# AndrewCullacino/handwritten-chinese-ocr-samples

Hardware: AMD Instinct MI355X
Metric: text-lines/sec (1x128x2000 synth) greedy decode (higher is better)
Workload: dtype f16 (f32 accumulate); 1 GPU; BASELINE configs[1]: 64 x 1x128x2000 uint8 lines, random-init hctr checkpoint (C=7358), forward + greedy CTC decode, labels to host; global_lines=64, lines_per_gpu=64, width=2000, classes=7358, checkpoint=random, parallelism=batch-shard x1

## Files before the change

handwritten-chinese-ocr-samples_amd/csrc/kernels.hip:

```cpp
#include "kernels.h"

#include <algorithm>
#include <climits>
#include <cstdlib>

namespace hctr {

typedef _Float16 f16x8 __attribute__((ext_vector_type(8)));
typedef float f32x4 __attribute__((ext_vector_type(4)));
typedef float f32x2 __attribute__((ext_vector_type(2)));
typedef _Float16 f16x2 __attribute__((ext_vector_type(2)));
typedef uint32_t u32x4 __attribute__((ext_vector_type(4)));
typedef void __attribute__((address_space(3))) * lptr_t;

__device__ __forceinline__ void glds16_asm(const char* gsrc, char* lds_dst) {
    const uint32_t lds = (uint32_t)(uintptr_t)((lptr_t)lds_dst);
    uint32_t keep;
    asm volatile("s_mov_b32 %0, m0\n\ts_mov_b32 m0, %2\n\ts_nop 0\n\tglobal_load_lds_dwordx4 %1, off\n\ts_mov_b32 m0, %0"
                 : "=&s"(keep)
                 : "v"(gsrc), "s"(lds)
                 : "memory");
}

template <int CTRL>
// ... 562 lines not shown
#pragma unroll
                    for (int n = 0; n < 4; ++n) dst[n] = *(const f16x8*)(xt + n * 2048 + (ks ? foff1 : foff0));
                };
                __builtin_amdgcn_sched_barrier(0);
                read_b(0, bq[0]);
                read_a(0, ar[0]);
                __builtin_amdgcn_sched_barrier(0);
                read_a(1, ar[1]);
                __builtin_amdgcn_sched_barrier(0);
                if (k + 1 < nk) stage(k + 1, (k + 1) & 1);
                __builtin_amdgcn_sched_barrier(0);
#pragma unroll
                for (int g = 0; g < 8; ++g) {
                    if (g + 2 < 8) read_a(g + 2, ar[(g + 2) % 3]);
                    __builtin_amdgcn_sched_barrier(0);
                    if (g == 1) { read_b(1, bq[1]); __builtin_amdgcn_sched_barrier(0); }
                    __builtin_amdgcn_s_setprio(1);
#pragma unroll
                    for (int jj = 0; jj < 2; ++jj)
#pragma unroll
                        for (int n = 0; n < 4; ++n)
                            acc[2 * (g & 3) + jj][n] = __builtin_amdgcn_mfma_f32_16x16x32_f16(ar[g % 3][jj], bq[g >> 2][n],
                                                                                             acc[2 * (g & 3) + jj][n], 0, 0, 0);
                    __builtin_amdgcn_s_setprio(0);
                    __builtin_amdgcn_sched_barrier(0);
                }
                continue;
            }
            if (k + 1 < nk) stage(k + 1, (k + 1) & 1);
#pragma unroll
            for (int ks = 0; ks < 2; ++ks) {
                const int fo = ks ? foff1 : foff0;
                f16x8 af[JT], bf[4];
#pragma unroll
                for (int n = 0; n < 4; ++n) bf[n] = *(const f16x8*)(xt + n * 2048 + fo);
#pragma unroll
                for (int j = 0; j < JT; ++j) af[j] = *(const f16x8*)(wt + j * 2048 + fo);
                __builtin_amdgcn_s_setprio(1);
#pragma unroll
                for (int j = 0; j < JT; ++j)
#pragma unroll
                    for (int n = 0; n < 4; ++n)
                        acc[j][n] = __builtin_amdgcn_mfma_f32_16x16x32_f16(af[j], bf[n], acc[j][n], 0, 0, 0);
                __builtin_amdgcn_s_setprio(0);
            }
        }
    } else {
        constexpr int NG = 2 * JT;
        constexpr int NP = NIW + NIX;
        for (int k = 0; k < nk; ++k) {
            asm volatile("s_waitcnt vmcnt(0)" ::: "memory");
            __syncthreads();
            const int kn = k + 1 < nk ? k + 1 : k;
            int64_t wo_n, xo_n;
            step_offsets(kn, wo_n, xo_n);
            const char* wsrc_n = wbase + wo_n;
            const char* xsrc_n = xbase + xo_n;
            const int buf_n = (k + 1) & 1;
            const char* wt = smem + (k & 1) * TILE_BYTES + (wn * WC) * 128;
            const char* xt = smem + (k & 1) * TILE_BYTES + BN * 128 + (wm * 64) * 128;
            f16x8 bfr[2][4], afr[2];
#pragma unroll
            for (int n = 0; n < 4; ++n) bfr[0][n] = *(const f16x8*)(xt + n * 2048 + foff0);
            afr[0] = *(const f16x8*)(wt + foff0);
#pragma unroll
            for (int g = 0; g < NG; ++g) {
                const int ks = g / JT, j = g % JT;
                if (g + 1 < NG) {
                    const int ks1 = (g + 1) / JT, j1 = (g + 1) % JT;
                    afr[(g + 1) & 1] = *(const f16x8*)(wt + j1 * 2048 + (ks1 ? foff1 : foff0));
                }
                if (g == JT / 2) {
#pragma unroll
                    for (int n = 0; n < 4; ++n) bfr[1][n] = *(const f16x8*)(xt + n * 2048 + foff1);
                }
                if ((g * NP) / NG != ((g + 1) * NP) / NG)
                    stage_piece(wsrc_n, xsrc_n, buf_n, (g * NP) / NG);
#pragma unroll
                for (int n = 0; n < 4; ++n)
                    acc[j][n] = __builtin_amdgcn_mfma_f32_16x16x32_f16(afr[g & 1], bfr[ks][n], acc[j][n], 0, 0, 0);
                __builtin_amdgcn_sched_barrier(0);
            }
        }
    }

    conv_epilogue<WN, WM, JT, LINEAR, SPLIT>(a, acc, smem, tid, lane, wn, wm, n0, mt, img, th, tw,
                                             th * (4 * WM) + wm * 4, tw * kTileW);
}

static int env_dbg() {
    if (getenv("HCTR_DBG_LAYER")) return 0;
    const char* e = getenv("HCTR_DBG");
    return e ? atoi(e) : 0;
}

static hipError_t raise_lds_limit(const void* fn, int bytes, bool (&done)[64]) {
    int dev = 0;
    hipError_t e = hipGetDevice(&dev);
    if (e != hipSuccess) return e;
    if (dev < 0 || dev >= 64) return hipErrorInvalidDevice;
    if (done[dev]) return hipSuccess;
    e = hipFuncSetAttribute(fn, hipFuncAttributeMaxDynamicSharedMemorySize, bytes);
    if (e == hipSuccess) done[dev] = true;
    return e;
}

constexpr int kHaloCols = 20;
constexpr int kHaloRows = 18;
constexpr int kHaloBytes = kHaloRows * kHaloCols * 128;
constexpr int kHaloPieces = kHaloRows * kHaloCols / 8;
constexpr int kHaloLds = 2 * 32768 + 2 * kHaloBytes;

template <bool SPLIT>
__global__ __launch_bounds__(512) void conv3x3_halo_kernel(const ConvArgs a) {
    constexpr int WN = 2, WM = 4, JT = 8, BN = 256;
    extern __shared__ __attribute__((aligned(16))) char smem[];
    const int tid = threadIdx.x;
    const int lane = tid & 63;
    const int wv = __builtin_amdgcn_readfirstlane(tid >> 6);
    const int wn = wv / WM, wm = wv % WM;

    const int total = a.mtiles * a.ntiles;
    int lin;
    {
        const int id = blockIdx.x, xcd = id & 7, s = id >> 3;
        const int q = total >> 3, r = total & 7;
        lin = (xcd < r ? xcd * (q + 1) : r * (q + 1) + (xcd - r) * q) + s;
    }
    const int nt = lin % a.ntiles;
    const int mt = lin / a.ntiles;
    const int n0 = nt * BN;
    const int tw = mt % a.tilesW;
    const int t2 = mt / a.tilesW;
    const int th = t2 % a.tilesH;
    const int img = t2 / a.tilesH;
    const int cin = a.Cin;
    const int nkc = cin / kBK;

    const char* xbase = (const char*)(a.x + img * a.in_sb + (int64_t)(th * 16) * a.in_sh + (int64_t)(tw * 16) * cin);
    const char* wbase = (const char*)(a.w + (int64_t)n0 * cin);
    const bool loader = wv < 4;
    uint32_t woff[8], hoff[12];
#pragma unroll
    for (int i = 0; i < 8; ++i) {
        const int g = ((wv & 3) * 8 + i) * 64 + lane;
        const int row = g >> 3, cp = (g & 7) ^ (row & 7);
        woff[i] = (uint32_t)row * (uint32_t)cin * 2u + cp * 16;
    }
#pragma unroll
    for (int r = 0; r < 12; ++r) {
        const int piece = ((r >> 1) * 4 + (wv & 3)) * 2 + (r & 1);
        const int g = piece * 64 + lane;
        const int row = g >> 3, cp = (g & 7) ^ (row & 7);
        int hy = row / kHaloCols, hx = row - hy * kHaloCols;
        if (hx > 17) hx = 17;
        if (hy > 17) hy = 17;
        hoff[r] = ((uint32_t)hy * (uint32_t)a.in_sh + (uint32_t)hx * (uint32_t)cin) * 2u + cp * 16;
    }
    const int q = lane >> 4, c = lane & 15;
    const int aoff0 = c * 128 + (((0 + q) ^ (lane & 7)) << 4);
    const int aoff1 = c * 128 + (((4 + q) ^ (lane & 7)) << 4);

    auto stage_weights = [&](int kc, int tap, int buf) {
        const char* src = wbase + ((int64_t)tap * a.CoutPad * cin + (int64_t)kc * kBK) * 2;
        char* dst = smem + buf * 32768 + ((wv & 3) * 8) * 1024;
#pragma unroll
        for (int i = 0; i < 8; ++i)
            glds16_asm(src + woff[i], dst + i * 1024);
    };
    auto stage_halo_piece = [&](int kc, int buf, int piece, uint32_t off) {
        if (piece < kHaloPieces) {
            const char* src = xbase + (int64_t)kc * (kBK * 2);
            char* dst = smem + 65536 + buf * kHaloBytes + piece * 1024;
            glds16_asm(src + off, dst);
        }
    };

    f32x4 acc[JT][4];
#pragma unroll
    for (int j = 0; j < JT; ++j)
#pragma unroll
        for (int n = 0; n < 4; ++n) acc[j][n] = (f32x4){0.f, 0.f, 0.f, 0.f};

    if (loader) {
#pragma unroll
        for (int r = 0; r < 12; ++r) stage_halo_piece(0, 0, ((r >> 1) * 4 + wv) * 2 + (r & 1), hoff[r]);
        stage_weights(0, 0, 0);
    }

    for (int kc = 0; kc < nkc; ++kc) {
        const bool next_chunk = kc + 1 < nkc;
        const int hbuf = 65536 + (kc & 1) * kHaloBytes + (wm * 4) * (kHaloCols * 128);
#pragma unroll 1
        for (int tap = 0; tap < 9; ++tap) {
            const int k = kc * 9 + tap;
            if (tap >= 1 && tap <= 5 && next_chunk) asm volatile("s_waitcnt vmcnt(2)" ::: "memory");
            else asm volatile("s_waitcnt vmcnt(0)" ::: "memory");
            __builtin_amdgcn_s_barrier();
            asm volatile("" ::: "memory");
            const int tdy = tap / 3, dx = tap - tdy * 3 - 1;
            const int u = c + 1 + dx;
            const int v0 = u * 128 + (((q ^ (u & 7) ^ ((tdy & 1) << 2)) & 7) << 4);
            const char* hb = smem + hbuf + tdy * (kHaloCols * 128);
            const char* be = hb + v0;
            const char* bo = hb + (v0 ^ 64);
            const char* wt = smem + (k & 1) * 32768 + (wn * 128) * 128;
            f16x8 ar[3][2], bq[2][4];
            auto read_a = [&](int g, f16x8 (&dst)[2]) {
                const int ks = g >> 2, jp = g & 3;
                const char* base = wt + (ks ? aoff1 : aoff0);
                dst[0] = *(const f16x8*)(base + (2 * jp) * 2048);
                dst[1] = *(const f16x8*)(base + (2 * jp + 1) * 2048);
            };
            auto read_b = [&](int ks, f16x8 (&dst)[4]) {
#pragma unroll
                for (int n = 0; n < 4; ++n)
                    dst[n] = *(const f16x8*)((((n & 1) ^ ks) ? bo : be) + n * (kHaloCols * 128));
            };
            __builtin_amdgcn_sched_barrier(0);
            read_b(0, bq[0]);
            read_a(0, ar[0]);
            __builtin_amdgcn_sched_barrier(0);
            read_a(1, ar[1]);
            __builtin_amdgcn_sched_barrier(0);
            if (loader) {
                int kc1 = kc, tap1 = tap + 1;
                if (tap1 == 9) { tap1 = 0; kc1 = next_chunk ? kc + 1 : kc; }
                if (a.dbg == 1) { kc1 = 0; tap1 = 0; }
                if (a.dbg != 2) stage_weights(kc1, tap1, (k + 1) & 1);
                if (next_chunk && tap < 6 && a.dbg != 2) {
                    uint32_t h0 = hoff[0], h1 = hoff[1];
                    h0 = tap == 1 ? hoff[2] : h0;  h1 = tap == 1 ? hoff[3] : h1;
                    h0 = tap == 2 ? hoff[4] : h0;  h1 = tap == 2 ? hoff[5] : h1;
                    h0 = tap == 3 ? hoff[6] : h0;  h1 = tap == 3 ? hoff[7] : h1;
                    h0 = tap == 4 ? hoff[8] : h0;  h1 = tap == 4 ? hoff[9] : h1;
                    h0 = tap == 5 ? hoff[10] : h0; h1 = tap == 5 ? hoff[11] : h1;
                    const int p0 = (tap * 4 + wv) * 2;
                    const int kcs = a.dbg == 1 ? 0 : kc + 1;
                    stage_halo_piece(kcs, (kc + 1) & 1, p0, h0);
                    stage_halo_piece(kcs, (kc + 1) & 1, p0 + 1, h1);
                }
            }
            __builtin_amdgcn_sched_barrier(0);
#pragma unroll
            for (int g = 0; g < 8; ++g) {
                const int ks = g >> 2, jp = g & 3;
                if (g + 2 < 8) read_a(g + 2, ar[(g + 2) % 3]);
                __builtin_amdgcn_sched_barrier(0);
                if (g == 1) { read_b(1, bq[1]); __builtin_amdgcn_sched_barrier(0); }
                __builtin_amdgcn_s_setprio(1);
#pragma unroll
                for (int jj = 0; jj < 2; ++jj)
#pragma unroll
                    for (int n = 0; n < 4; ++n)
                        acc[2 * jp + jj][n] = __builtin_amdgcn_mfma_f32_16x16x32_f16(ar[g % 3][jj], bq[ks][n],
                                                                                    acc[2 * jp + jj][n], 0, 0, 0);
                __builtin_amdgcn_s_setprio(0);
                __builtin_amdgcn_sched_barrier(0);
            }
        }
    }
    asm volatile("s_waitcnt vmcnt(0)" ::: "memory");
    conv_epilogue<WN, WM, JT, false, SPLIT>(a, acc, smem, tid, lane, wn, wm, n0, mt, img, th, tw, th * 16 + wm * 4,
                                            tw * 16);
}

namespace halo4_lds {
constexpr int kWeightBuf = 16384;
constexpr int kWeights = 0;
constexpr int kHalo = kWeights + 2 * kWeightBuf;
constexpr int kScratch = kHalo + kHaloBytes;
constexpr int kScratchBytes = 4 * 128 * 4;
constexpr int kHaloTable = kScratch;
constexpr int kHaloTableBytes = 4 * 12 * 8 * 4;
constexpr int kNextTile = kScratch + kScratchBytes;
constexpr int kTotal = kNextTile + 16;
static_assert(kHaloTableBytes <= kScratchBytes, "the halo-offset table fits inside the epilogue scratch it aliases");
static_assert(kNextTile >= kScratch + kScratchBytes, "the next-tile words lie behind the epilogue scratch");
static_assert(kTotal <= 80 * 1024, "two workgroups per CU on 160 KB of LDS");
}

template <int GEOM, bool SPLIT, bool PERSIST, bool STAMP = false, bool DSFUSE = false, bool RESPRE = false>
__global__ __launch_bounds__(256, 2) void conv3x3_halo4_kernel(const ConvArgs a) {
    static_assert(!DSFUSE || !PERSIST, "downsample fusion: non-persistent instances only");
    static_assert(!RESPRE || (!DSFUSE && !PERSIST && !SPLIT), "residual-in-prologue: plain f16 instances only");
    constexpr int WN = 1, WM = 4, JT = 8, BN = 128;
    constexpr int TR = GEOM ? 8 : 16, TC = GEOM ? 32 : 16;
    constexpr int S = TC + 4;
    static_assert((TR + 2) * S * 128 == kHaloBytes, "halo footprint");
    extern __shared__ __attribute__((aligned(16))) char smem[];
    const int tid = threadIdx.x;
    auto stamp = [&](int i) {
        if (STAMP && tid == 0) a.stamps[(size_t)blockIdx.x * 16 + i] = __builtin_amdgcn_s_memrealtime();
    };
    stamp(0);
    const int lane = tid & 63;
    const int wv = __builtin_amdgcn_readfirstlane(tid >> 6);
    const int wm = wv;
    const int cin = a.Cin;
    const int nkc = (a.dbg & 64) ? 0 : cin / kBK;
    const int nk = 9 * nkc;
    constexpr bool kPrefetch = !PERSIST && !STAMP && !RESPRE;
    static_assert(!(kPrefetch && PERSIST), "the halo-offset table aliases the epilogue scratch: one tile per workgroup");
    constexpr int kRing = 3;
    constexpr int kBhalfAt = 1;
    constexpr int kBpreAt = 4;
    constexpr int kEarlyAt = 1;

    {
        const int k0 = a.mtiles, k1 = a.ntiles, k2 = a.tilesW, k3 = a.tilesH, k4 = a.Cin, k5 = a.in_sh, k6 = a.nt_shift,
                  k7 = a.th_shift, k8 = a.CoutPad;
        const uint64_t k9 = a.tw_magic;
        const int64_t k10 = a.in_sb;
        const half_t *k11 = a.x, *k12 = a.w;
        const float* k13 = a.bias;
        asm volatile("" ::"s"(k0), "s"(k1), "s"(k2), "s"(k3), "s"(k4), "s"(k5), "s"(k6), "s"(k7), "s"(k8), "s"(k9), "s"(k10),
                     "s"(k11), "s"(k12), "s"(k13));
    }
    const int total = a.mtiles * a.ntiles;
    const int xcd = blockIdx.x & 7, local = blockIdx.x >> 3;
    const int tq = total >> 3, tr = total & 7;
    const int xbase_lin = xcd < tr ? xcd * (tq + 1) : tr * (tq + 1) + (xcd - tr) * tq;
    const int xcnt = tq + (xcd < tr ? 1 : 0);
    const int nloc = PERSIST ? (int)(gridDim.x >> 3) : 1;
    struct Tile { int n0, mt, img, th, tw; const char* xb; const char* wb; };
    auto tile_at = [&](int idx) {
        Tile t;
        const int lin = xbase_lin + idx;
        int nt, t2, th, img;
        if (a.nt_shift >= 0) { nt = lin & (a.ntiles - 1); t.mt = lin >> a.nt_shift; }
        else { nt = lin % a.ntiles; t.mt = lin / a.ntiles; }
        t.n0 = nt * BN;
        t2 = (int)(((uint64_t)(uint32_t)t.mt * a.tw_magic) >> 40);
        const int tw = t.mt - t2 * a.tilesW;
        if (a.th_shift >= 0) { th = t2 & (a.tilesH - 1); img = t2 >> a.th_shift; }
        else { th = t2 % a.tilesH; img = t2 / a.tilesH; }
        t.img = img; t.th = th; t.tw = tw;
        t.xb = (const char*)(a.x + img * a.in_sb + (int64_t)(th * TR) * a.in_sh + (int64_t)(tw * TC) * cin);
        t.wb = (const char*)(a.w + (int64_t)t.n0 * cin);
        return t;
    };
    int tidx = local;
    if (PERSIST && tidx >= xcnt) return;
    const bool dynamic = PERSIST && a.tile_counter != nullptr;
    int tnext = local + nloc;
    volatile int* lds_next = (volatile int*)(smem + halo4_lds::kNextTile);

    const int wrow = GEOM ? (wm >> 1) * 4 : wm * 4;
    const int wcol = GEOM ? (wm & 1) * 16 : 0;
    uint32_t woff[4], hoff[12];
    const int q = lane >> 4, c = lane & 15;
    const int aoff0 = c * 128 + (((0 + q) ^ (lane & 7)) << 4);
    const int aoff1 = c * 128 + (((4 + q) ^ (lane & 7)) << 4);

    auto weight_buf = [&](int k) { return smem + halo4_lds::kWeights + (k & 1) * halo4_lds::kWeightBuf; };
    auto stage_w = [&](const char* wb, int rowcin, const uint32_t (&wo)[4], int kc, int tap, int buf) {
        const char* src = wb + ((int64_t)tap * a.CoutPad * rowcin + (int64_t)kc * kBK) * 2;
        char* dst = weight_buf(buf) + (wv * 4) * 1024;
        const int64_t ps = (int64_t)rowcin * 16;
        glds16x4_asm_s(src, src + ps, src + 2 * ps, src + 3 * ps, wo[0], dst, dst + 1024, dst + 2048, dst + 3072);
    };
    auto stage_weights = [&](const char* wb, int kc, int tap, int buf) { stage_w(wb, cin, woff, kc, tap, buf); };
    auto stage_halo = [&](const char* xb, int kc) {
        const char* src = xb + (int64_t)kc * (kBK * 2);
#pragma unroll
        for (int r = 0; r < 12; ++r)
            if (wv + 4 * r < kHaloPieces) glds16_asm_s(src, hoff[r], smem + halo4_lds::kHalo + (wv + 4 * r) * 1024);
    };
    auto lane_offsets = [&](int rowcin, int in_sh, uint32_t (&wo)[4], bool with_halo) {
        int ln = lane;
        asm volatile("" : "+v"(ln));
#pragma unroll
        for (int i = 0; i < 4; ++i) {
            const int g = (wv * 4 + i) * 64 + ln;
            const int row = g >> 3, cp = (g & 7) ^ (row & 7);
            wo[i] = (uint32_t)row * (uint32_t)rowcin * 2u + cp * 16;
        }
        if (!with_halo) return;
#pragma unroll
        for (int r = 0; r < 12; ++r) {
            const int g = (wv + 4 * r) * 64 + ln;
            const int row = g >> 3, cp = (g & 7) ^ (row & 7);
            int hy = row / S, hx = row - hy * S;
            if (hx > TC + 1) hx = TC + 1;
            if (hy > TR + 1) hy = TR + 1;
            hoff[r] = ((uint32_t)hy * (uint32_t)in_sh + (uint32_t)hx * (uint32_t)rowcin) * 2u + cp * 16;
        }
    };
    auto write_halo_table = [&]() {
        uint32_t* htab = (uint32_t*)(smem + halo4_lds::kHaloTable);
        if ((lane & 7) == 0) {
            const uint32_t cp0 = (uint32_t)((lane >> 3) & 7) << 4;
#pragma unroll
            for (int r = 0; r < 12; ++r) htab[(wv * 12 + r) * 8 + (lane >> 3)] = hoff[r] - cp0;
        }
    };
    const int hbuf = halo4_lds::kHalo + wrow * (S * 128);
    int bx[3][2];
#pragma unroll
    for (int d = 0; d < 3; ++d) {
        const int u = wcol + c + d;
        const int v0 = u * 128 + (((q ^ (u & 7)) & 7) << 4);
        bx[d][0] = hbuf + v0;
        bx[d][1] = hbuf + (v0 ^ 64);
    }
    auto b_ptrs = [&](int tap, const char*& be, const char*& bo) {
        const int tdy = tap / 3, d = tap - tdy * 3;
        be = smem + bx[d][tdy & 1] + tdy * (S * 128);
        bo = smem + bx[d][(tdy & 1) ^ 1] + tdy * (S * 128);
    };

    Tile cur = tile_at(tidx);
    int kbase = 0;
    bool first = true;

    int tile_no = 0;
    for (;;) {
        const bool has_next = PERSIST && (tnext < xcnt);
        const char* nxb = cur.xb;
        const char* nwb = cur.wb;
        if (has_next) {
            const Tile t = tile_at(tnext);
            nxb = t.xb;
            nwb = t.wb;
        }
        int drawn = 0;
        if (dynamic && tid == 0)
            drawn = 2 * nloc + __hip_atomic_fetch_add(a.tile_counter + xcd, 1, __ATOMIC_RELAXED, __HIP_MEMORY_SCOPE_AGENT);
        f32x4 acc[JT][4];
        f16x8 bq[2][4];
        auto mma_step = [&](const char* wt, const char* be, const char* bo, auto&& stage_next, auto&& after_group,
                            bool have_b0 = false, const char* nbe = nullptr, const char* nbo = nullptr,
                            int bhalf_at = kBhalfAt) {
            f16x8 ar[kRing][2];
            auto read_a = [&](int g, f16x8 (&dst)[2]) {
                const int ks = g >> 2, jp = g & 3;
                const char* base = wt + (ks ? aoff1 : aoff0);
                dst[0] = *(const f16x8*)(base + (2 * jp) * 2048);
                dst[1] = *(const f16x8*)(base + (2 * jp + 1) * 2048);
            };
            auto read_b = [&](int ks, f16x8 (&dst)[4]) {
#pragma unroll
                for (int n = 0; n < 4; ++n)
                    dst[n] = *(const f16x8*)((((n & 1) ^ ks) ? bo : be) + n * (S * 128));
            };
            __builtin_amdgcn_sched_barrier(0);
            if (!have_b0) read_b(0, bq[0]);
            read_a(0, ar[0]);
            __builtin_amdgcn_sched_barrier(0);
#pragma unroll
            for (int g = 1; g < kRing - 1; ++g) read_a(g, ar[g]);
            __builtin_amdgcn_sched_barrier(0);
            stage_next();
            __builtin_amdgcn_sched_barrier(0);
#pragma unroll
            for (int g = 0; g < 8; ++g) {
                const int ks = g >> 2, jp = g & 3;
                if (g + kRing - 1 < 8) read_a(g + kRing - 1, ar[(g + kRing - 1) % kRing]);
                __builtin_amdgcn_sched_barrier(0);
                if (g == bhalf_at) { read_b(1, bq[1]); __builtin_amdgcn_sched_barrier(0); }
#pragma unroll
                for (int jj = 0; jj < 2; ++jj)
#pragma unroll
                    for (int n = 0; n < 4; ++n)
                        acc[2 * jp + jj][n] = __builtin_amdgcn_mfma_f32_16x16x32_f16(
                            ar[g % kRing][jj], bq[ks][n], acc[2 * jp + jj][n], 0, 0, 0);
                if (g == kBpreAt && nbe != nullptr) {
#pragma unroll
                    for (int n = 0; n < 4; ++n) bq[0][n] = *(const f16x8*)(((n & 1) ? nbo : nbe) + n * (S * 128));
                }
                after_group(g);
                __builtin_amdgcn_sched_barrier(0);
            }
        };

        if (DSFUSE) {
            const int dcin = a.ds_cin, nds = dcin / kBK;
            const int tw0 = cur.tw, th0 = cur.th, img0 = cur.img;
            const char* dxb = (const char*)(a.ds_x + img0 * a.ds_in_sb + (int64_t)(th0 * TR) * a.ds_in_sh +
                                            (int64_t)(tw0 * TC) * dcin);
            const char* dwb = (const char*)(a.ds_w + (int64_t)cur.n0 * dcin);
            uint32_t woff_x[4];
            lane_offsets(dcin, a.ds_in_sh, woff_x, true);
            lane_offsets(cin, a.in_sh, woff, false);
            stage_halo(dxb, 0);
            stage_w(dwb, dcin, woff_x, 0, 0, 0);
            __builtin_amdgcn_s_setprio(1);
#pragma unroll
            for (int j = 0; j < JT; ++j)
#pragma unroll
                for (int n = 0; n < 4; ++n) acc[j][n] = (f32x4){0.f, 0.f, 0.f, 0.f};
            __builtin_amdgcn_s_waitcnt(0xc07f);
#pragma unroll 1
            for (int kc = 0; kc < nds; ++kc) {
                asm volatile("s_waitcnt vmcnt(0)" ::: "memory");
                __builtin_amdgcn_s_barrier();
                asm volatile("" ::: "memory");
                const char *be, *bo;
                b_ptrs(4, be, bo);
                mma_step(weight_buf(kc), be, bo, [&] {
                    if (kc + 1 < nds) stage_w(dwb, dcin, woff_x, kc + 1, 0, (kc + 1) & 1);
                    else stage_w(cur.wb, cin, woff, 0, 0, (kc + 1) & 1);
                }, [&](int) {});
                __builtin_amdgcn_s_barrier();
                asm volatile("" ::: "memory");
                if (kc + 1 < nds) {
                    stage_halo(dxb, kc + 1);
                } else {
                    lane_offsets(cin, a.in_sh, woff, true);
                    stage_halo(cur.xb, 0);
                    if (kPrefetch) write_halo_table();
                }
            }
            kbase = nds;
            const float* sc = a.se_scale + (int64_t)img0 * a.Cout + cur.n0 + q * 8;
#pragma unroll
            for (int j = 0; j < JT; ++j) {
                const int o = acc_cout_offset(j);
                const f32x4 bd = *(const f32x4*)(a.ds_bias + cur.n0 + q * 8 + o);
                const f32x4 b2 = *(const f32x4*)(a.bias + cur.n0 + q * 8 + o);
                const f32x4 s4 = *(const f32x4*)(sc + o);
#pragma unroll
                for (int i = 0; i < 4; ++i) {
                    const float inv = __builtin_amdgcn_rcpf(fmaxf(s4[i], kSeScaleFloor));
#pragma unroll
                    for (int n = 0; n < 4; ++n) acc[j][n][i] = fmaf(acc[j][n][i] + bd[i], inv, b2[i]);
                }
            }
        } else {
            if (PERSIST || first) lane_offsets(cin, a.in_sh, woff, true);
            if (first) {
                stage_halo(cur.xb, 0);
                stage_weights(cur.wb, 0, 0, 0);
                if (kPrefetch) write_halo_table();
                first = false;
                if (STAMP) {
                    stamp(1);
                    asm volatile("s_waitcnt vmcnt(0)" ::: "memory");
                    __builtin_amdgcn_s_barrier();
                    stamp(2);
                }
            }
            if (RESPRE) {
                const int w = cur.tw * TC + wcol + c;
                const bool wok = w < a.out_wlimit;
                const half_t* rb = a.resid + a.out_off + cur.img * a.out_sb + (int64_t)w * a.out_sw + cur.n0 + q * 8 +
                                   (int64_t)(cur.th * TR + wrow) * a.out_sh;
                const float* sc = a.se_scale + (int64_t)cur.img * a.Cout + cur.n0 + q * 8;
                f16x8 rlo[JT / 4][4], rhi[JT / 4][4];
#pragma unroll
                for (int cb = 0; cb < JT / 4; ++cb)
#pragma unroll
                    for (int n = 0; n < 4; ++n) {
                        const half_t* r = rb + (int64_t)n * a.out_sh + cb * 64;
                        rlo[cb][n] = wok ? *(const f16x8*)r : (f16x8){0, 0, 0, 0, 0, 0, 0, 0};
                        rhi[cb][n] = wok ? *(const f16x8*)(r + 32) : (f16x8){0, 0, 0, 0, 0, 0, 0, 0};
                    }
#pragma unroll
                for (int j = 0; j < JT; ++j) {
                    const f32x4 b4 = *(const f32x4*)(a.bias + cur.n0 + q * 8 + acc_cout_offset(j));
                    const f32x4 s4 = *(const f32x4*)(sc + acc_cout_offset(j));
#pragma unroll
                    for (int i = 0; i < 4; ++i) {
                        const float inv = __builtin_amdgcn_rcpf(fmaxf(s4[i], kSeScaleFloor));
                        const int e = (j & 3) * 4 + i;
#pragma unroll
                        for (int n = 0; n < 4; ++n) {
                            const float r = e < 8 ? (float)rlo[j >> 2][n][e] : (float)rhi[j >> 2][n][e - 8];
                            acc[j][n][i] = fmaf(r, inv, b4[i]);
                        }
                    }
                }
            } else {
#pragma unroll
                for (int j = 0; j < JT; ++j) {
                    const f32x4 b4 = *(const f32x4*)(a.bias + cur.n0 + q * 8 + acc_cout_offset(j));
#pragma unroll
                    for (int n = 0; n < 4; ++n) acc[j][n] = b4;
                }
            }
        }

        __builtin_amdgcn_s_waitcnt(0xc07f);
        __builtin_amdgcn_s_setprio(1);
        for (int kc = 0; kc < nkc; ++kc) {
            const bool next_chunk = kc + 1 < nkc;
#pragma unroll
            for (int tap = 0; tap < 9; ++tap) {
                const int k = kc * 9 + tap;
                asm volatile("s_waitcnt vmcnt(0)" ::: "memory");
                if (!(a.dbg & 1024)) __builtin_amdgcn_s_barrier();
                asm volatile("" ::: "memory");
                const char *be, *bo;
                b_ptrs(tap, be, bo);
                const bool more = k + 1 < nk;
                const bool wrap = tap == 8;
                const int tap1 = more ? (wrap ? 0 : tap + 1) : 0;
                const int kc1 = more ? (wrap ? kc + 1 : kc) : 0;
                const char* wsrc = more ? cur.wb : nwb;
                const char *nbe = nullptr, *nbo = nullptr;
                if (kPrefetch && tap < 8) b_ptrs(tap + 1, nbe, nbo);
                mma_step(weight_buf(kbase + k), be, bo, [&] {
                    if ((more || has_next) && !(a.dbg & 512))
                        stage_weights(wsrc, kc1, tap1, (kbase + k + 1) & 1);
                }, [&](int g) {
                    if (kPrefetch && tap == 8 && g == kEarlyAt && next_chunk) {
                        asm volatile("s_waitcnt lgkmcnt(0)" ::: "memory");
                        __builtin_amdgcn_s_barrier();
                        asm volatile("" ::: "memory");
                        static_assert(kHaloPieces == 45, "halo piece count");
                        const char* hsrc = (next_chunk ? cur.xb + (int64_t)(kc + 1) * (kBK * 2) : nxb);
                        char* d = smem + halo4_lds::kHalo + wv * 1024;
                        int ln = lane;
                        asm volatile("" : "+v"(ln));
                        const uint32_t* hrow = (const uint32_t*)(smem + halo4_lds::kHaloTable) + wv * 96 + (ln >> 3);
                        const uint32_t cpl = (uint32_t)((ln ^ (ln >> 3)) & 7) << 4;
                        uint32_t ho[4];
#pragma unroll
                        for (int r = 0; r < 4; ++r) ho[r] = hrow[r * 8] + cpl;
                        glds16x4v_asm_s<4096>(hsrc, ho[0], ho[1], ho[2], ho[3], d);
#pragma unroll
                        for (int r = 0; r < 4; ++r) ho[r] = hrow[(4 + r) * 8] + cpl;
                        glds16x4v_asm_s<4096>(hsrc, ho[0], ho[1], ho[2], ho[3], d + 4 * 4096);
#pragma unroll
                        for (int r = 0; r < 4; ++r) ho[r] = hrow[(8 + r) * 8] + cpl;
#pragma unroll
                        for (int r = 8; r < 11; ++r) glds16_asm_s(hsrc, ho[r - 8], d + r * 4096);
                        if (wv == 0) glds16_asm_s(hsrc, ho[3], d + 11 * 4096);
                    }
                }, kPrefetch && tap > 0, nbe, nbo, (kPrefetch && tap == 8) ? 0 : kBhalfAt);
            }
            if (!kPrefetch && (next_chunk || has_next) && !(a.dbg & 32)) {
                __builtin_amdgcn_s_barrier();
                asm volatile("" ::: "memory");
                if (next_chunk) stage_halo(cur.xb, kc + 1);
                else stage_halo(nxb, 0);
            }
        }
        __builtin_amdgcn_s_setprio(0);
        stamp(3);
        if (a.dbg & 128) {
            float t = 0.f;
#pragma unroll
            for (int j = 0; j < JT; ++j)
#pragma unroll
                for (int n = 0; n < 4; ++n) t += acc[j][n][0] + acc[j][n][1] + acc[j][n][2] + acc[j][n][3];
            if (t == 123.456f) ((half_t*)a.y)[0] = (half_t)t;
        } else
        {
            const int tw = cur.tw, th = cur.th, img = cur.img;
            conv_epilogue<WN, WM, JT, false, SPLIT, true, true, DSFUSE || RESPRE>(
                a, acc, smem + halo4_lds::kScratch, tid, lane, 0, wm, cur.n0, cur.mt, img, th, tw, th * TR + wrow,
                tw * TC + wcol, STAMP ? a.stamps + (size_t)blockIdx.x * 16 : nullptr);
        }
        if (!has_next) break;
        kbase += nk;
        tidx = tnext;
        if (dynamic) {
            if (tid == 0) lds_next[tile_no & 1] = drawn;
            __builtin_amdgcn_s_waitcnt(0xc07f);
            __builtin_amdgcn_s_barrier();
            tnext = __builtin_amdgcn_readfirstlane(lds_next[tile_no & 1]);
        } else {
            tnext = tidx + nloc;
        }
        ++tile_no;
        cur = tile_at(tidx);
    }
    if (a.dbg & 64) asm volatile("s_waitcnt vmcnt(0)" ::: "memory");
    if (STAMP) {
        stamp(4);
        asm volatile("s_waitcnt vmcnt(0)" ::: "memory");
        stamp(5);
        if (tid == 0) {
            a.stamps[(size_t)blockIdx.x * 16 + 6] = __builtin_amdgcn_s_getreg((31 << 11) | 4);
            a.stamps[(size_t)blockIdx.x * 16 + 7] = __builtin_amdgcn_s_getreg((31 << 11) | 20);
        }
    }
}

template <int GEOM>
__global__ __launch_bounds__(256, 2) void conv3x3_halo4h_kernel(const ConvArgs a) {
    constexpr int WN = 1, WM = 4, JT = 8, BN = 128;
    constexpr int TR = GEOM ? 8 : 16, TC = GEOM ? 32 : 16;
    constexpr int S = TC + 4;
    constexpr int kHalf = (TR + 2) * S * 64;
    constexpr int kHalfPieces = (kHalf + 1023) / 1024;
    static_assert(2 * kHalf == kHaloBytes && kHalfPieces == 23, "halo footprint");
    extern __shared__ __attribute__((aligned(16))) char smem[];
    const int tid = threadIdx.x;
    const int lane = tid & 63;
    const int wv = __builtin_amdgcn_readfirstlane(tid >> 6);
    const int wm = wv;
    const int cin = a.Cin;
    const int nkc = cin / kBK;
    {
        const int k0 = a.mtiles, k1 = a.ntiles, k2 = a.tilesW, k3 = a.tilesH, k4 = a.Cin, k5 = a.in_sh, k6 = a.nt_shift,
                  k7 = a.th_shift, k8 = a.CoutPad;
        const uint64_t k9 = a.tw_magic;
        const int64_t k10 = a.in_sb;
        const half_t *k11 = a.x, *k12 = a.w;
        const float* k13 = a.bias;
        asm volatile("" ::"s"(k0), "s"(k1), "s"(k2), "s"(k3), "s"(k4), "s"(k5), "s"(k6), "s"(k7), "s"(k8), "s"(k9), "s"(k10),
                     "s"(k11), "s"(k12), "s"(k13));
    }
    const int total = a.mtiles * a.ntiles;
    const int xcd = blockIdx.x & 7, local = blockIdx.x >> 3;
    const int tq = total >> 3, tr = total & 7;
    const int lin = (xcd < tr ? xcd * (tq + 1) : tr * (tq + 1) + (xcd - tr) * tq) + local;
    int nt, mt, t2, th, img;
    if (a.nt_shift >= 0) { nt = lin & (a.ntiles - 1); mt = lin >> a.nt_shift; }
    else { nt = lin % a.ntiles; mt = lin / a.ntiles; }
    const int n0 = nt * BN;
    t2 = (int)(((uint64_t)(uint32_t)mt * a.tw_magic) >> 40);
    const int tw = mt - t2 * a.tilesW;
    if (a.th_shift >= 0) { th = t2 & (a.tilesH - 1); img = t2 >> a.th_shift; }
    else { th = t2 % a.tilesH; img = t2 / a.tilesH; }
    const char* xb = (const char*)(a.x + img * a.in_sb + (int64_t)(th * TR) * a.in_sh + (int64_t)(tw * TC) * cin);
    const char* wb = (const char*)(a.w + (int64_t)n0 * cin);

    const int wrow = GEOM ? (wm >> 1) * 4 : wm * 4;
    const int wcol = GEOM ? (wm & 1) * 16 : 0;
    const int q = lane >> 4, c = lane & 15;
    uint32_t woff0;
    {
        int ln = lane;
        asm volatile("" : "+v"(ln));
        const int prow = ln >> 2, slot = ln & 3;
        const int row = ((wv * 4) & 7) * 16 + prow;
        woff0 = (uint32_t)row * (uint32_t)cin * 2u + (uint32_t)((slot ^ (((row >> 2) & 1) << 1)) << 4);
    }
    const int wpiece = 16 * cin * 2;
    auto stage_w = [&](int kc, int s, int buf) {
        const int u = 2 * s + (wv >> 1);
        const int tap = u < 9 ? u : u - 9, half = u < 9 ? 0 : 1;
        const char* src = wb + ((int64_t)tap * a.CoutPad * cin + (int64_t)kc * kBK + half * 32) * 2;
        char* dst = smem + halo4_lds::kWeights + buf * halo4_lds::kWeightBuf + (wv * 4) * 1024;
#pragma unroll
        for (int i = 0; i < 4; ++i) glds16_asm_s(src + i * wpiece, woff0, dst + i * 1024);
    };
    auto stage_h2 = [&](int kc, int half, int r0) {
        const char* src = xb + ((int64_t)kc * kBK + half * 32) * 2;
        char* dst = smem + halo4_lds::kHalo + half * kHalf;
        int ln = lane;
        asm volatile("" : "+v"(ln));
        const int prow = ln >> 2, slot = ln & 3;
#pragma unroll
        for (int rr = 0; rr < 2; ++rr) {
            const int r = r0 + rr;
            int hp = wv + 4 * r;
            if (hp > kHalfPieces - 1) hp = kHalfPieces - 1;
            const int hr = hp * 16 + prow;
            int hy = (int)(((uint32_t)hr * (65536u / S + 1u)) >> 16), hx = hr - hy * S;
            if (hx > TC + 1) hx = TC + 1;
            if (hy > TR + 1) hy = TR + 1;
            const uint32_t off = ((uint32_t)hy * (uint32_t)a.in_sh + (uint32_t)hx * (uint32_t)cin) * 2u +
                                 (uint32_t)((slot ^ (((hr >> 2) & 1) << 1)) << 4);
            if (hp == kHalfPieces - 1) {
                if (lane < 32) glds16_asm_s(src, off, dst + hp * 1024);
            } else {
                glds16_asm_s(src, off, dst + hp * 1024);
            }
        }
    };
    const int aoff = c * 64 + ((q ^ (((c >> 2) & 1) << 1)) << 4);

    stage_h2(0, 0, 0);
    stage_h2(0, 0, 2);
    stage_h2(0, 0, 4);
    stage_w(0, 0, 0);
    f32x4 acc[JT][4];
#pragma unroll
    for (int j = 0; j < JT; ++j) {
        const f32x4 b4 = *(const f32x4*)(a.bias + n0 + q * 8 + acc_cout_offset(j));
#pragma unroll
        for (int n = 0; n < 4; ++n) acc[j][n] = b4;
    }
    __builtin_amdgcn_s_waitcnt(0xc07f);
    __builtin_amdgcn_s_setprio(1);
    int gstep = 0;
    bool halo_prev = false;
    for (int kc = 0; kc < nkc; ++kc) {
        const bool next_chunk = kc + 1 < nkc;
#pragma unroll
        for (int s = 0; s < 9; ++s, ++gstep) {
            if (halo_prev) asm volatile("s_waitcnt vmcnt(2)" ::: "memory");
            else asm volatile("s_waitcnt vmcnt(0)" ::: "memory");
            __builtin_amdgcn_s_barrier();
            asm volatile("" ::: "memory");
            const char* wt = smem + halo4_lds::kWeights + (gstep & 1) * halo4_lds::kWeightBuf + aoff;
            const char *be[2], *bo[2];
#pragma unroll
            for (int uu = 0; uu < 2; ++uu) {
                const int u = 2 * s + uu;
                const int tap = u < 9 ? u : u - 9, half = u < 9 ? 0 : 1;
                const int tdy = tap / 3, dx = tap - tdy * 3 - 1;
                const int hr0 = (wrow + tdy) * S + wcol + c + 1 + dx;
                const char* hb = smem + halo4_lds::kHalo + half * kHalf + hr0 * 64;
                const int slot = q ^ (((hr0 >> 2) & 1) << 1);
                be[uu] = hb + (slot << 4);
                bo[uu] = hb + ((slot ^ 2) << 4);
            }
            const bool more = !(s == 8 && !next_chunk);
            const bool halo_now = (s < 3) || (next_chunk && s >= 5 && s < 8);
            f16x8 ar[3][2], bq[2][4];
            auto read_a = [&](int g, f16x8 (&dst)[2]) {
                const char* base = wt + (g >> 2) * 8192 + (2 * (g & 3)) * 1024;
                dst[0] = *(const f16x8*)base;
                dst[1] = *(const f16x8*)(base + 1024);
            };
            auto read_b = [&](int uu, f16x8 (&dst)[4]) {
#pragma unroll
                for (int n = 0; n < 4; ++n) dst[n] = *(const f16x8*)(((n & 1) ? bo[uu] : be[uu]) + n * (S * 64));
            };
            __builtin_amdgcn_sched_barrier(0);
            read_b(0, bq[0]);
            read_a(0, ar[0]);
            __builtin_amdgcn_sched_barrier(0);
            read_a(1, ar[1]);
            __builtin_amdgcn_sched_barrier(0);
            if (more) {
                const int s1 = s == 8 ? 0 : s + 1, kc1 = s == 8 ? kc + 1 : kc;
                stage_w(kc1, s1, (gstep + 1) & 1);
            }
            if (halo_now) {
                if (s < 3) stage_h2(kc, 1, 2 * s);
                else stage_h2(kc + 1, 0, 2 * (s - 5));
            }
            halo_prev = halo_now;
            __builtin_amdgcn_sched_barrier(0);
#pragma unroll
            for (int g = 0; g < 8; ++g) {
                if (g + 2 < 8) read_a(g + 2, ar[(g + 2) % 3]);
                __builtin_amdgcn_sched_barrier(0);
                if (g == 1) { read_b(1, bq[1]); __builtin_amdgcn_sched_barrier(0); }
#pragma unroll
                for (int jj = 0; jj < 2; ++jj)
#pragma unroll
                    for (int n = 0; n < 4; ++n)
                        acc[2 * (g & 3) + jj][n] = __builtin_amdgcn_mfma_f32_16x16x32_f16(ar[g % 3][jj], bq[g >> 2][n],
                                                                                         acc[2 * (g & 3) + jj][n], 0, 0, 0);
                __builtin_amdgcn_sched_barrier(0);
            }
        }
    }
    __builtin_amdgcn_s_setprio(0);
    conv_epilogue<WN, WM, JT, false, false, true, true, false>(a, acc, smem + halo4_lds::kScratch, tid, lane, 0, wm, n0, mt, img, th, tw,
                                                               th * TR + wrow, tw * TC + wcol);
}

template <auto KERNEL>
static hipError_t launch_halo4_instance(const ConvArgs& a0, int grid, hipStream_t s, bool with_env_dbg = true) {
    static bool done[64] = {};
    hipError_t e0 = raise_lds_limit((const void*)KERNEL, halo4_lds::kTotal, done);
    if (e0 != hipSuccess) return e0;
    static const int dbg = env_dbg();
    ConvArgs a = a0;
    if (with_env_dbg) a.dbg |= dbg;
    hipLaunchKernelGGL(KERNEL, dim3(grid), dim3(256), halo4_lds::kTotal, s, a);
    return hipGetLastError();
}

template <int GEOM, bool SPLIT, bool PERSIST>
static hipError_t launch_conv_halo4_tp(const ConvArgs& a, hipStream_t s) {
    int grid = a.mtiles * a.ntiles;
    if (PERSIST) {
        static int cus[64] = {};
        int dev = 0;
        (void)hipGetDevice(&dev);
        if (dev >= 0 && dev < 64 && cus[dev] == 0) {
            hipDeviceProp_t prop;
            if (hipGetDeviceProperties(&prop, dev) == hipSuccess) cus[dev] = prop.multiProcessorCount;
            if (cus[dev] <= 0) cus[dev] = 256;
        }
        const int resident = 2 * ((dev >= 0 && dev < 64) ? cus[dev] : 256);
        if (grid > resident) grid = resident;
        grid = (grid + 7) / 8 * 8;
    }
    return launch_halo4_instance<conv3x3_halo4_kernel<GEOM, SPLIT, PERSIST>>(a, grid, s);
}
template <int GEOM, bool SPLIT>
static hipError_t launch_conv_halo4_t(const ConvArgs& a, hipStream_t s) {
    const int grid = a.mtiles * a.ntiles;
    if (a.ds_x != nullptr) {
        if (GEOM != 0) return hipErrorInvalidValue;
        return launch_halo4_instance<conv3x3_halo4_kernel<0, SPLIT, false, false, true>>(a, grid, s);
    }
    if (a.stamps != nullptr && !SPLIT)
        return launch_halo4_instance<conv3x3_halo4_kernel<GEOM, false, false, true>>(a, grid, s, false);
    static const int persist = [] { const char* e = getenv("HCTR_PERSIST"); return e ? atoi(e) : 0; }();
    if constexpr (!SPLIT) {
        static const int respre = [] { const char* e = getenv("HCTR_RESPRE"); return e ? atoi(e) : 0; }();
        if (respre && persist == 0 && a.resid != nullptr && a.se_scale != nullptr)
            return launch_halo4_instance<conv3x3_halo4_kernel<GEOM, false, false, false, false, true>>(a, grid, s);
    }
    if (persist == 0 || (persist == 2 && a.tile_counter == nullptr)) return launch_conv_halo4_tp<GEOM, SPLIT, false>(a, s);
    ConvArgs b = a;
    if (persist != 2) b.tile_counter = nullptr;
    return launch_conv_halo4_tp<GEOM, SPLIT, true>(b, s);
}
template <int GEOM>
static hipError_t launch_conv_halo4(const ConvArgs& a0, hipStream_t s) {
    ConvArgs a = a0;
    auto shift_of = [](int v) { int sft = 0; while ((1 << sft) < v) ++sft; return (1 << sft) == v ? sft : -1; };
    a.nt_shift = shift_of(a.ntiles);
    a.th_shift = shift_of(a.tilesH);
    if (a.tilesW < 1 || (uint64_t)a.mtiles * (uint64_t)a.tilesW >= ((uint64_t)1 << 40)) return hipErrorInvalidValue;
    a.tw_magic = (((uint64_t)1 << 40) + (uint64_t)a.tilesW - 1) / (uint64_t)a.tilesW;
    static const bool halfhalo = [] { const char* e = getenv("HCTR_HALFHALO"); return e ? atoi(e) != 0 : false; }();
    static const int persist = [] { const char* e = getenv("HCTR_PERSIST"); return e ? atoi(e) : 0; }();
    if (halfhalo && !a.split && a.ds_x == nullptr && a.stamps == nullptr && persist == 0 && a.Cin % kBK == 0)
        return launch_halo4_instance<conv3x3_halo4h_kernel<GEOM>>(a, a.mtiles * a.ntiles, s);
    return a.split ? launch_conv_halo4_t<GEOM, true>(a, s) : launch_conv_halo4_t<GEOM, false>(a, s);
}

template <bool SPLIT>
static hipError_t launch_conv_halo_t(const ConvArgs& a, hipStream_t s) {
    static bool done[64] = {};
    hipError_t e0 = raise_lds_limit((const void*)conv3x3_halo_kernel<SPLIT>, kHaloLds, done);
    if (e0 != hipSuccess) return e0;
    static const int dbg = env_dbg();
    ConvArgs b = a;
    b.dbg |= dbg;
    hipLaunchKernelGGL(conv3x3_halo_kernel<SPLIT>, dim3(a.mtiles * a.ntiles), dim3(512), kHaloLds, s, b);
    return hipGetLastError();
}
static hipError_t launch_conv_halo(const ConvArgs& a, hipStream_t s) {
    return a.split ? launch_conv_halo_t<true>(a, s) : launch_conv_halo_t<false>(a, s);
}

size_t conv_lds_bytes(ConvTile tile) {
    switch (tile) {
        case TILE_64x256: return 2 * (64 + 256) * 128;
// ... 3873 lines not shown
```

Before: 508.1 lines/s.

## Reorder conv taps column-major and slide B fragments across vertical taps

Reorders the 3x3 conv tap loop so that the three vertical taps of each horizontal offset run consecutively. When prefetching is on, B fragments held in registers are reused through a rotating index, and only the one new row is loaded from LDS per vertical step instead of all four. The weight-staging tap index is remapped to match the new order. This cuts LDS read traffic in the implicit-GEMM mainloop, in exchange for more complex register indexing and inline-asm xor addressing.

```diff
diff --git a/handwritten-chinese-ocr-samples_amd/csrc/kernels.hip b/handwritten-chinese-ocr-samples_amd/csrc/kernels.hip
--- a/handwritten-chinese-ocr-samples_amd/csrc/kernels.hip
+++ b/handwritten-chinese-ocr-samples_amd/csrc/kernels.hip
@@ -888,6 +888,7 @@
     const int nk = 9 * nkc;
     constexpr bool kPrefetch = !PERSIST && !STAMP && !RESPRE;
     static_assert(!(kPrefetch && PERSIST), "the halo-offset table aliases the epilogue scratch: one tile per workgroup");
+    constexpr bool kSlide = kPrefetch && !SPLIT;
     constexpr int kRing = 3;
     constexpr int kBhalfAt = 1;
     constexpr int kBpreAt = 4;
@@ -990,10 +991,12 @@
         bx[d][0] = hbuf + v0;
         bx[d][1] = hbuf + (v0 ^ 64);
     }
-    auto b_ptrs = [&](int tap, const char*& be, const char*& bo) {
-        const int tdy = tap / 3, d = tap - tdy * 3;
-        be = smem + bx[d][tdy & 1] + tdy * (S * 128);
-        bo = smem + bx[d][(tdy & 1) ^ 1] + tdy * (S * 128);
+    static_assert(halo4_lds::kHalo % 128 == 0, "bx[d][1] == bx[d][0] ^ 64");
+    auto frag_b = [&](int d, int r, int ks) {
+        if (!kSlide) return *(const f16x8*)(smem + bx[d][(r ^ ks) & 1] + r * (S * 128));
+        int ad = bx[d][0];
+        if ((r ^ ks) & 1) asm volatile("v_xor_b32 %0, 64, %1" : "=v"(ad) : "v"(bx[d][0]));
+        return *(const f16x8*)(smem + ad + r * (S * 128));
     };
 
     Tile cur = tile_at(tidx);
@@ -1015,9 +1018,9 @@
             drawn = 2 * nloc + __hip_atomic_fetch_add(a.tile_counter + xcd, 1, __ATOMIC_RELAXED, __HIP_MEMORY_SCOPE_AGENT);
         f32x4 acc[JT][4];
         f16x8 bq[2][4];
-        auto mma_step = [&](const char* wt, const char* be, const char* bo, auto&& stage_next, auto&& after_group,
-                            bool have_b0 = false, const char* nbe = nullptr, const char* nbo = nullptr,
-                            int bhalf_at = kBhalfAt) {
+        auto mma_step = [&](const char* wt, int d, int dy, bool slide, auto&& stage_next, auto&& after_group,
+                            bool have_b0 = false, bool pre = false, int bhalf_at = kBhalfAt) {
+            const int rot = slide ? dy : 0;
             f16x8 ar[kRing][2];
             auto read_a = [&](int g, f16x8 (&dst)[2]) {
                 const int ks = g >> 2, jp = g & 3;
@@ -1025,13 +1028,13 @@
                 dst[0] = *(const f16x8*)(base + (2 * jp) * 2048);
                 dst[1] = *(const f16x8*)(base + (2 * jp + 1) * 2048);
             };
-            auto read_b = [&](int ks, f16x8 (&dst)[4]) {
-#pragma unroll
-                for (int n = 0; n < 4; ++n)
-                    dst[n] = *(const f16x8*)((((n & 1) ^ ks) ? bo : be) + n * (S * 128));
+            auto read_b = [&](int ks, int sd, int sdy) {
+                const int srot = slide ? sdy : 0;
+#pragma unroll
+                for (int n = (slide && sdy > 0) ? 3 : 0; n < 4; ++n) bq[ks][(n + srot) & 3] = frag_b(sd, sdy + n, ks);
             };
             __builtin_amdgcn_sched_barrier(0);
-            if (!have_b0) read_b(0, bq[0]);
+            if (!have_b0) read_b(0, d, dy);
             read_a(0, ar[0]);
             __builtin_amdgcn_sched_barrier(0);
 #pragma unroll
@@ -1044,16 +1047,16 @@
                 const int ks = g >> 2, jp = g & 3;
                 if (g + kRing - 1 < 8) read_a(g + kRing - 1, ar[(g + kRing - 1) % kRing]);
                 __builtin_amdgcn_sched_barrier(0);
-                if (g == bhalf_at) { read_b(1, bq[1]); __builtin_amdgcn_sched_barrier(0); }
+                if (g == bhalf_at) { read_b(1, d, dy); __builtin_amdgcn_sched_barrier(0); }
 #pragma unroll
                 for (int jj = 0; jj < 2; ++jj)
 #pragma unroll
                     for (int n = 0; n < 4; ++n)
                         acc[2 * jp + jj][n] = __builtin_amdgcn_mfma_f32_16x16x32_f16(
-                            ar[g % kRing][jj], bq[ks][n], acc[2 * jp + jj][n], 0, 0, 0);
-                if (g == kBpreAt && nbe != nullptr) {
-#pragma unroll
-                    for (int n = 0; n < 4; ++n) bq[0][n] = *(const f16x8*)(((n & 1) ? nbo : nbe) + n * (S * 128));
+                            ar[g % kRing][jj], bq[ks][(n + rot) & 3], acc[2 * jp + jj][n], 0, 0, 0);
+                if (g == kBpreAt && pre) {
+                    if (dy < 2) read_b(0, d, dy + 1);
+                    else read_b(0, d + 1, 0);
                 }
                 after_group(g);
                 __builtin_amdgcn_sched_barrier(0);
@@ -1082,9 +1085,7 @@
                 asm volatile("s_waitcnt vmcnt(0)" ::: "memory");
                 __builtin_amdgcn_s_barrier();
                 asm volatile("" ::: "memory");
-                const char *be, *bo;
-                b_ptrs(4, be, bo);
-                mma_step(weight_buf(kc), be, bo, [&] {
+                mma_step(weight_buf(kc), 1, 1, false, [&] {
                     if (kc + 1 < nds) stage_w(dwb, dcin, woff_x, kc + 1, 0, (kc + 1) & 1);
                     else stage_w(cur.wb, cin, woff, 0, 0, (kc + 1) & 1);
                 }, [&](int) {});
@@ -1172,25 +1173,24 @@
         for (int kc = 0; kc < nkc; ++kc) {
             const bool next_chunk = kc + 1 < nkc;
 #pragma unroll
-            for (int tap = 0; tap < 9; ++tap) {
-                const int k = kc * 9 + tap;
+            for (int t = 0; t < 9; ++t) {
+                const int d = t / 3, dy = t - d * 3;
+                const int k = kc * 9 + t;
                 asm volatile("s_waitcnt vmcnt(0)" ::: "memory");
                 if (!(a.dbg & 1024)) __builtin_amdgcn_s_barrier();
                 asm volatile("" ::: "memory");
-                const char *be, *bo;
-                b_ptrs(tap, be, bo);
                 const bool more = k + 1 < nk;
-                const bool wrap = tap == 8;
-                const int tap1 = more ? (wrap ? 0 : tap + 1) : 0;
+                const bool wrap = t == 8;
+                const int t1 = more ? (wrap ? 0 : t + 1) : 0;
+                const int tap1 = (t1 % 3) * 3 + t1 / 3;
                 const int kc1 = more ? (wrap ? kc + 1 : kc) : 0;
                 const char* wsrc = more ? cur.wb : nwb;
-                const char *nbe = nullptr, *nbo = nullptr;
-                if (kPrefetch && tap < 8) b_ptrs(tap + 1, nbe, nbo);
-                mma_step(weight_buf(kbase + k), be, bo, [&] {
+                const int bhalf_at = kPrefetch ? (t == 8 ? 0 : kBhalfAt) : ((kSlide && dy > 0) ? 0 : kBhalfAt);
+                mma_step(weight_buf(kbase + k), d, dy, kSlide, [&] {
                     if ((more || has_next) && !(a.dbg & 512))
                         stage_weights(wsrc, kc1, tap1, (kbase + k + 1) & 1);
                 }, [&](int g) {
-                    if (kPrefetch && tap == 8 && g == kEarlyAt && next_chunk) {
+                    if (kPrefetch && t == 8 && g == kEarlyAt && next_chunk) {
                         asm volatile("s_waitcnt lgkmcnt(0)" ::: "memory");
                         __builtin_amdgcn_s_barrier();
                         asm volatile("" ::: "memory");
@@ -1214,7 +1214,7 @@
                         for (int r = 8; r < 11; ++r) glds16_asm_s(hsrc, ho[r - 8], d + r * 4096);
                         if (wv == 0) glds16_asm_s(hsrc, ho[3], d + 11 * 4096);
                     }
-                }, kPrefetch && tap > 0, nbe, nbo, (kPrefetch && tap == 8) ? 0 : kBhalfAt);
+                }, kPrefetch && t > 0, kPrefetch && t < 8, bhalf_at);
             }
             if (!kPrefetch && (next_chunk || has_next) && !(a.dbg & 32)) {
                 __builtin_amdgcn_s_barrier();
```

New measurement: 511.6 lines/s (median of 6 runs). Within noise of the previous version (+0.7%).
